# pujariaditya/WaveVerify

Hardware: AMD Instinct MI355X
Metric: clips/sec embed+detect, 1s@16kHz bs=256 (higher is better)
Workload: dtype f32; 1 GPU; embed_detect: 256 clips x 1 s @ 16 kHz per GPU (BASELINE.json configs[1]), seeded random weights; batch_per_gpu=256, global_batch=256, clip_samples=16000, parallelism=dp1 (independent clip shards, no data-path collective)

## Files before the change

include/waveverify_hip.h:

```cpp
#ifndef WAVEVERIFY_HIP_H
#define WAVEVERIFY_HIP_H

#include <stddef.h>
#include <stdint.h>

#ifdef __cplusplus
extern "C" {
#endif

#define WV_OK 0
#define WV_EINVAL (-1)
#define WV_ENOKEY (-2)
#define WV_EHIP (-3)
#define WV_ESTATE (-4)
#define WV_ENOMEM (-5)

#define WV_KIND_GENERATOR 0
#define WV_KIND_DETECTOR 1
#define WV_KIND_LOCATOR 2

#define WV_MAX_STRIDES 8

typedef struct wv_config {
    int32_t kind;
// ... 78 lines not shown
int wv_profile_collect(int index, char* name_out, int name_cap, int64_t* launches,
                       double* total_ms, double* flops, double* bytes);

int wv_window_gather(const float* src, int64_t n_src, const int64_t* offs, float* dst, int W, int L, void* stream);
int wv_window_scatter(const float* y, const int64_t* desc, float* out, int64_t n_out, int W, int C, int L, void* stream);
int wv_detector_forward_windowed(wv_model* m, const float* x, const int* keep_lo, const int* keep_hi, float* psum,
                                 int W, int L, void* workspace, size_t workspace_bytes, void* stream);
int wv_detector_forward_windowed_f16(wv_model* m, const float* x, const int* keep_lo, const int* keep_hi, float* psum,
                                     int W, int L, void* workspace, size_t workspace_bytes, void* stream);
int wv_window_reduce_mean(const float* psum, int n_rows, const int* ptr, const int* rows, const int64_t* lengths,
                          float* mean_prob, int B, int nb, void* stream);
int wv_frames_reduce(const float* fsum, int B, int nb, int Fr_stride, const int* seg, int n_seg, float eps, float* prob, double* count,
                     void* stream);
int wv_session_advance(const float* hist, int hcap, int hv, const float* x, int n, float* win, int wlen,
                       float* hist_out, int drop, int hv2, int S, void* stream);


int wv_op_pw_dw(const float* X, const float* w_pw, const float* w_dw, const float* dw_bias,
                const float* film, const float* resid, float* Y,
                int B, int K, int M, int Tin, int ks, int stride, int dilation,
                float pre_scale, int pre_elu, float out_scale, int bands,
                float* Yact, float act_scale, void* stream);

int wv_op_resblock(const float* X, float pre_scale, const float* w_pw1, const float* w_dw1, const float* b1,
                   const float* w_pw2, const float* w_dw2, const float* b2, float* Y, float* Yact,
                   int B, int C, int T, float out_scale, float act_scale, void* stream);

int wv_op_dw_pw(const float* X, const float* w_dw, const float* w_pw, const float* bias, float* Y,
                int B, int K, int M, int Tin, int mode, int ks_or_ratio,
                float pre_scale, int pre_elu, int l2norm, int accumulate, float out_scale,
                float* Yact, float act_scale, void* stream);

int wv_op_stft_logmag(const float* wav, const float* host_basis, float* P, int B, int T,
                      int n_fft, int hop, float mean, float std, void* stream);

int wv_op_spec_block(const float* wav, const float* basis_or_null, const float* w_pw, const float* x, float* Y, float* Yact, int B, int T,
                     int n_fft, int hop, int M, float mean, float std, float out_scale, float act_scale, void* stream);

int wv_op_conv_pre(const float* x, const float* w, const float* bias, float* Y, int B, int C,
                   int T, int ks, float in_scale, void* stream);

int wv_op_tail(const float* H, const float* w, const float* bias, const float* x_or_null,
               float* out, int B, int C, int Tin, int T, int ks, float pre_scale, float out_scale,
               void* stream);

int wv_op_head(const float* Z, const float* w_rev, const float* b_rev,
// ... 231 lines not shown
```

waveverify_amd/_lib.py:

```python
from __future__ import annotations

import ctypes as C
import os
from typing import Optional

HERE = os.path.dirname(os.path.abspath(__file__))
LIB_PATH = os.path.join(HERE, "lib", "libwaveverify_hip.so")
WV_MAX_STRIDES = 8

WV_KIND = {"generator": 0, "detector": 1, "locator": 2}


class WvConfig(C.Structure):
    _fields_ = [
        ("kind", C.c_int32), ("dimension", C.c_int32), ("msg_dimension", C.c_int32),
        ("channels_enc", C.c_int32), ("channels_dec", C.c_int32), ("n_fft_base", C.c_int32),
        ("n_residual_enc", C.c_int32), ("n_residual_dec", C.c_int32), ("n_strides", C.c_int32),
        ("strides", C.c_int32 * WV_MAX_STRIDES),
        ("kernel_size", C.c_int32), ("last_kernel_size", C.c_int32),
        ("residual_kernel_size", C.c_int32), ("dilation_base", C.c_int32),
        ("zero_init", C.c_int32), ("nbits", C.c_int32), ("output_dim", C.c_int32),
        ("embedding_dim", C.c_int32), ("embedding_layers", C.c_int32), ("freq_bands", C.c_int32),
        ("res_scale_enc", C.c_float), ("res_scale_dec", C.c_float), ("wav_std", C.c_float),
        ("spec_means", C.c_float * (WV_MAX_STRIDES + 1)),
# ... 10 lines not shown
    "wv_config_default": (C.c_int, [C.c_int, C.POINTER(WvConfig)]),
    "wv_model_create": (C.c_int, [C.POINTER(WvConfig), C.POINTER(_VP)]),
    "wv_model_destroy": (None, [_VP]),
    "wv_model_num_params": (C.c_int, [_VP]),
    "wv_model_param_info": (C.c_int, [_VP, C.c_int, C.c_char_p, C.c_int, C.POINTER(C.c_int64),
                                      C.POINTER(C.c_int), C.POINTER(C.c_int)]),
    "wv_model_set_param": (C.c_int, [_VP, C.c_char_p, _VP, C.c_int64]),
    "wv_model_set_param_wn": (C.c_int, [_VP, C.c_char_p, _VP, C.c_int64, _VP, C.c_int64]),
    "wv_model_set_stft_basis": (C.c_int, [_VP, C.c_char_p, _VP, C.c_int64]),
    "wv_model_finalize": (C.c_int, [_VP]),
    "wv_workspace_bytes": (C.c_size_t, [_VP, C.c_int, C.c_int]),
    "wv_generator_forward": (C.c_int, [_VP, _VP, _VP, C.c_int, _VP, C.c_int, C.c_int, C.c_int,
                                       _VP, C.c_size_t, _VP]),
    "wv_detector_forward": (C.c_int, [_VP, _VP, _VP, _VP, C.c_int, C.c_int, _VP, C.c_size_t, _VP]),
    "wv_locator_forward": (C.c_int, [_VP, _VP, _VP, C.c_int, C.c_int, _VP, C.c_size_t, _VP]),
    "wv_encoder_forward": (C.c_int, [_VP, _VP, _VP, C.c_int, _VP, C.c_int, C.c_int, _VP,
                                     C.c_size_t, _VP]),
    "wv_detector_forward_f16": (C.c_int, [_VP, _VP, _VP, _VP, C.c_int, C.c_int, _VP, C.c_size_t, _VP]),
    "wv_detector_forward_frames": (C.c_int, [_VP, _VP, _VP, C.c_float, _VP, C.c_int, C.c_int, _VP, C.c_size_t, _VP]),
    "wv_detector_forward_frames_f16": (C.c_int, [_VP, _VP, _VP, C.c_float, _VP, C.c_int, C.c_int, _VP, C.c_size_t, _VP]),
    "wv_locator_forward_f16": (C.c_int, [_VP, _VP, _VP, C.c_int, C.c_int, _VP, C.c_size_t, _VP]),
    "wv_generator_forward_f16": (C.c_int, [_VP, _VP, _VP, C.c_int, _VP, C.c_int, C.c_int, C.c_int, _VP, C.c_size_t, _VP]),
    "wv_model_film": (C.c_int, [_VP, _VP, C.c_int, _VP, C.c_int, _VP]),
    "wv_profile_enable": (C.c_int, [C.c_int]),
    "wv_profile_reset": (C.c_int, []),
    "wv_profile_collect": (C.c_int, [C.c_int, C.c_char_p, C.c_int, C.POINTER(C.c_int64),
                                     C.POINTER(C.c_double), C.POINTER(C.c_double),
                                     C.POINTER(C.c_double)]),
    "wv_window_gather": (C.c_int, [_VP, C.c_int64, _VP, _VP, C.c_int, C.c_int, _VP]),
    "wv_window_scatter": (C.c_int, [_VP, _VP, _VP, C.c_int64, C.c_int, C.c_int, C.c_int, _VP]),
    "wv_detector_forward_windowed": (C.c_int, [_VP, _VP, _VP, _VP, _VP, C.c_int, C.c_int, _VP, C.c_size_t, _VP]),
    "wv_detector_forward_windowed_f16": (C.c_int, [_VP, _VP, _VP, _VP, _VP, C.c_int, C.c_int, _VP, C.c_size_t, _VP]),
    "wv_window_reduce_mean": (C.c_int, [_VP, C.c_int, _VP, _VP, _VP, _VP, C.c_int, C.c_int, _VP]),
    "wv_frames_reduce": (C.c_int, [_VP, C.c_int, C.c_int, C.c_int, _VP, C.c_int, C.c_float, _VP, _VP, _VP]),
    "wv_session_advance": (C.c_int, [_VP, C.c_int, C.c_int, _VP, C.c_int, _VP, C.c_int, _VP, C.c_int, C.c_int, C.c_int, _VP]),
    "wv_op_pw_dw": (C.c_int, [_VP, _VP, _VP, _VP, _VP, _VP, _VP, C.c_int, C.c_int, C.c_int,
                              C.c_int, C.c_int, C.c_int, C.c_int, C.c_float, C.c_int, C.c_float,
                              C.c_int, _VP, C.c_float, _VP]),
    "wv_op_resblock": (C.c_int, [_VP, C.c_float] + [_VP] * 8 + [C.c_int, C.c_int, C.c_int, C.c_float, C.c_float, _VP]),
    "wv_op_dw_pw": (C.c_int, [_VP, _VP, _VP, _VP, _VP, C.c_int, C.c_int, C.c_int, C.c_int, C.c_int,
                              C.c_int, C.c_float, C.c_int, C.c_int, C.c_int, C.c_float, _VP, C.c_float, _VP]),
    "wv_op_stft_logmag": (C.c_int, [_VP, _VP, _VP, C.c_int, C.c_int, C.c_int, C.c_int, C.c_float,
                                    C.c_float, _VP]),
    "wv_op_spec_block": (C.c_int, [_VP] * 6 + [C.c_int] * 5 + [C.c_float] * 4 + [_VP]),
    "wv_op_conv_pre": (C.c_int, [_VP, _VP, _VP, _VP, C.c_int, C.c_int, C.c_int, C.c_int,
                                 C.c_float, _VP]),
# ... 174 lines not shown
```

waveverify_amd/csrc/wv_k1.hip:

```cpp
#include <algorithm>
#include <atomic>
#include <cstdlib>
#include <string>
#include <type_traits>

#include "wv_dev.h"

namespace wv {

typedef const __attribute__((address_space(1))) void* gptr_t;
typedef __attribute__((address_space(3))) void* lptr_t;

__device__ __attribute__((aligned(16))) float g_zero16[4] = {0.f, 0.f, 0.f, 0.f};

__device__ __forceinline__ float dpp_next(float v) {
    return __builtin_bit_cast(float, __builtin_amdgcn_update_dpp(0, __builtin_bit_cast(int, v), 0x130, 0xf, 0xf, true));
}

template <int NT_, int BKC_, int BM_ = 128>
struct K1 {
    static constexpr int NT = NT_, BN = 32 * NT_, BKC = BKC_, KQ = BKC_ / 4, BM = BM_, WM = BM_ / 32, NTHREADS = 64 * WM;
    static constexpr int A4 = KQ * BM;
    static constexpr int B4 = BKC * BN / 4;
    static constexpr int STAGE4 = A4 + B4;
    static constexpr int A_PIECES = A4 / 64, B_PIECES = B4 / 64;
    static constexpr int A_PER = (A_PIECES + WM - 1) / WM, B_PER_DMA = (B_PIECES + WM - 1) / WM;
    static constexpr int CG = BN / 4;
    static constexpr int HLD = BN + 4;
    static constexpr int NBT = (BKC / 2) * CG;
    static constexpr int B_PER = (NBT + NTHREADS - 1) / NTHREADS;
    static_assert(A4 % 64 == 0 && B4 % 64 == 0 && NTHREADS % CG == 0 && 64 % CG == 0, "staging maps");
};

template <int NT> struct NVec;
template <> struct NVec<4> { typedef f32x4 type; };
template <> struct NVec<2> { typedef f32x2 type; };

constexpr int OOB_VOFF = 0x40000000;

template <class C>
struct DmaRows {
    const float* src; size_t ld; int K; int rbase;
    __device__ __forceinline__ void init(const float* Xb, int K_, int Tin, int ti0, int wave, int lane) {
        const int col = ti0 + 4 * (lane % C::CG);
        rbase = lane / C::CG;
        const bool inr = col >= 0 && col + 3 < Tin;
        src = inr ? Xb + col : g_zero16;
        ld = inr ? (size_t)Tin : 0;
        K = K_;
        (void)wave;
    }
    __device__ __forceinline__ void init_flat(const float* X, int K_, int Tin, int B, int Tv, int pad, long long g0, int lane) {
        const long long g = g0 + 4 * (lane % C::CG);
        const int b = (int)(g / Tv), t = (int)(g - (long long)b * Tv) - pad;
        rbase = lane / C::CG;
        const bool inr = b < B && t >= 0;
        src = inr ? X + (size_t)b * K_ * Tin + t : g_zero16;
        ld = inr ? (size_t)Tin : 0;
        K = K_;
    }
    __device__ __forceinline__ void issue(int c, f32x4* Bst, int wave) const {
#pragma unroll
        for (int i = 0; i < C::B_PER_DMA; ++i) {
            const int pi = wave + i * C::WM;
            if (C::B_PIECES % C::WM == 0 || pi < C::B_PIECES) {
                const int k = min(c * C::BKC + pi * (64 / C::CG) + rbase, K - 1);
                __builtin_amdgcn_global_load_lds((gptr_t)(src + (size_t)k * ld), (lptr_t)(Bst + pi * 64), 16, 0, 0);
            }
        }
    }
};

template <class C>
struct DmaA {
    __amdgpu_buffer_rsrc_t rsrc;
    int voff[C::A_PER];
    int chunk_bytes;
    __device__ __forceinline__ void init(const f32x4* wq, int Mp, int m0, int nchunks, int wave, int lane) {
        rsrc = __builtin_amdgcn_make_buffer_rsrc(const_cast<f32x4*>(wq + m0), 0, (nchunks * C::KQ * Mp - m0) * 16, 0x00020000);
        chunk_bytes = C::KQ * Mp * 16;
#pragma unroll
        for (int i = 0; i < C::A_PER; ++i) {
            const int idx = (wave + i * C::WM) * 64 + lane;
            voff[i] = ((idx / C::BM) * Mp + idx % C::BM) * 16;
        }
    }
    __device__ __forceinline__ void issue(int c, f32x4* Ast, int wave) const {
        const int soff = c * chunk_bytes;
#pragma unroll
        for (int i = 0; i < C::A_PER; ++i) {
            const int pi = wave + i * C::WM;
// ... 82 lines not shown
        voff0 = act_lane ? ((m0 + 32 * wave + 4 * half) * p.Tout + to) * 4 : 0x7f000000;
        if (EPI == 0 && p.flat) {
            const long long gc = gflat + p.pad + o;
            const int bo2 = (int)(gc / p.Tv), t = (int)(gc - (long long)bo2 * p.Tv) - p.pad;
            const bool ok = o < p.tto && bo2 < p.B && t >= 0;
            Yb = p.Y; Ab = p.Yact; Rb = HASR ? p.resid : nullptr; Rb2 = RES == 2 ? p.resid2 : nullptr; Hb = RAWH ? p.Yraw : nullptr; Sb = RES == 5 ? p.Ysum : nullptr;
            nrec = (int)((long long)p.B * M * p.Tout * 4);
            voff0 = ok ? (int)((((long long)bo2 * M + m0 + 32 * wave + 4 * half) * p.Tout + t) * 4) : (int)0x80000000u;
        }
        if (EPI == 8 && p.flat) {
            const int TvO = p.Tv >> 3;
            const long long go = gflat / 8 + (q >> 1);
            const int bo2 = (int)(go / TvO), n = (int)(go - (long long)bo2 * TvO);
            const bool ok = (q & 1) == 0 && (q >> 1) < p.tto && bo2 < p.B && n < p.Tout;
            Yb = p.Y; Ab = p.Yact;
            nrec = (int)((long long)p.B * M * p.Tout * 4);
            voff0 = ok ? (int)((((long long)bo2 * M + m0 + 32 * wave + 4 * half) * p.Tout + n) * 4) : (int)0x80000000u;
            fgam = 1.f; fbet = 0.f;
            if (p.film) {
                const float* fl = p.film + (size_t)min(bo2, p.B - 1) * p.film_stride + 2 * (m0 / (M / p.bands));
                fgam = fl[0]; fbet = fl[1];
            }
        }
        const bool lane_film = EPI == 8 && p.flat;
        const int bw = p.film ? (M / p.bands) : 1;
        const float* filmb = (p.film && !lane_film) ? p.film + (size_t)b * p.film_stride : nullptr;
        for (int m = tid; m < C::BM; m += C::NTHREADS) {
            const int gm = m0 + m;
            float* row = Wl + m * WLD;
#pragma unroll
            for (int i = 0; i < NTAP; ++i) row[i] = (gm < M && i < p.ks) ? p.dw_w[(size_t)gm * p.ks + i] : 0.f;
            float gam = 1.f, bet = 0.f;
            if (filmb && gm < M) { const int band = gm / bw; gam = filmb[2 * band]; bet = filmb[2 * band + 1]; }
            row[NTAP] = (gm < M && p.dw_b) ? p.dw_b[gm] : 0.f;
            row[NTAP + 1] = gam; row[NTAP + 2] = bet;
            if (EPI != 0) row[WLD - 1] = 0.f;
        }
    }

    typedef unsigned uvec __attribute__((ext_vector_type(NT)));
    __device__ __forceinline__ ovec buf_load(__amdgpu_buffer_rsrc_t r, int off) const {
        if constexpr (NT == 4) return __builtin_bit_cast(ovec, __builtin_amdgcn_raw_buffer_load_b128(r, off, 0, 0));
        else return __builtin_bit_cast(ovec, __builtin_amdgcn_raw_buffer_load_b64(r, off, 0, 0));
    }
    __device__ __forceinline__ void buf_store(__amdgpu_buffer_rsrc_t r, int off, ovec v) const {
        if constexpr (NT == 4) __builtin_amdgcn_raw_buffer_store_b128(__builtin_bit_cast(uvec, v), r, off, 0, 0);
        else __builtin_amdgcn_raw_buffer_store_b64(__builtin_bit_cast(uvec, v), r, off, 0, 0);
    }

    __device__ __forceinline__ void finish(f32x16 (&acc)[NT], const PwDwArgs& p, float* strips) {
        if constexpr (EPI == 0) {
            constexpr int NSH = 4 / NT;
            const int clip_bytes = nrec;
            const __amdgpu_buffer_rsrc_t rY = uniform_rsrc(Yb ? Yb : p.Yact, Yb ? clip_bytes : 0);
            const __amdgpu_buffer_rsrc_t rA = uniform_rsrc(Ab ? Ab : p.Yact, Ab ? clip_bytes : 0);
            const __amdgpu_buffer_rsrc_t rR = uniform_rsrc(Rb ? Rb : p.X, Rb ? clip_bytes : 0);
            const int row_bytes = p.Tout * 4;
            const int voff = voff0;
            const float* Wrow = Wl + (32 * wave + 4 * half) * 8;
            ovec res4[HASR ? 4 : 1];
            ovec add4[RES == 2 ? 4 : 1];
            const __amdgpu_buffer_rsrc_t rR2 = uniform_rsrc(Rb2 ? Rb2 : p.X, Rb2 ? clip_bytes : 0);
            const __amdgpu_buffer_rsrc_t rH = uniform_rsrc(Hb ? Hb : p.Y, Hb ? clip_bytes : 0);
            const __amdgpu_buffer_rsrc_t rS = uniform_rsrc(Sb ? Sb : p.Y, Sb ? clip_bytes : 0);
            const float sres = (RES == 5 && p.scale_ptr) ? p.out_scale * p.scale_ptr[0] : p.out_scale;
            if constexpr (HASR) {
#pragma unroll
                for (int r = 0; r < 4; ++r) res4[r] = buf_load(rR, voff + ((r & 3) + 8 * (r >> 2)) * row_bytes);
            }
            if constexpr (RES == 2) {
#pragma unroll
                for (int r = 0; r < 4; ++r) add4[r] = buf_load(rR2, voff + ((r & 3) + 8 * (r >> 2)) * row_bytes);
            }
            f32x4 w0n = *reinterpret_cast<const f32x4*>(Wrow), w1n = *reinterpret_cast<const f32x4*>(Wrow + 4);
#pragma unroll
            for (int r = 0; r < 16; ++r) {
                const int cr = (r & 3) + 8 * (r >> 2);
                const f32x4 w0 = w0n, w1 = w1n;
                if (r + 1 < 16) {
                    const int cn = ((r + 1) & 3) + 8 * ((r + 1) >> 2);
                    w0n = *reinterpret_cast<const f32x4*>(Wrow + cn * 8);
                    w1n = *reinterpret_cast<const f32x4*>(Wrow + cn * 8 + 4);
                }
                float hh[NT + 4], cur[NT];
#pragma unroll
                for (int e = 0; e < NT; ++e) { cur[e] = acc[e][r]; hh[e] = cur[e]; }
#pragma unroll
                for (int s2 = 1; s2 <= NSH; ++s2) {
#pragma unroll
                    for (int e = 0; e < NT; ++e) { cur[e] = dpp_next(cur[e]); hh[s2 * NT + e] = cur[e]; }
                }
                const int off = voff + cr * row_bytes;
                ovec y;
#pragma unroll
                for (int e = 0; e < NT; ++e) {
                    float v = fmaf(w0.x, hh[e], w1.y);
// ... 157 lines not shown
template <> struct LdrSel<4> { typedef ConvTrPair<1> type; };
template <> struct LdrSel<5> { typedef ConvTrPair<0> type; };
template <> struct LdrSel<6> { typedef ConvTrLds<4> type; };
template <> struct LdrSel<7> { typedef ConvTrLds<2> type; };
template <class C> constexpr int k1_lwp(int ldr) { return ldr == 7 ? (C::BN / 2 + 6 + 3) / 4 * 4 : (C::BN / 4 + 6 + 3) / 4 * 4; }

template <class C, int EPI, int LDR, int RES, int NS>
__global__ __launch_bounds__(C::NTHREADS, LDR >= 2 ? (C::B_PER > 1 ? 2 : 3) : 4) void k1_kernel(PwDwArgs p) {
    extern __shared__ __attribute__((aligned(16))) float smem[];
    constexpr bool REG = LDR != 0;
    typedef K1Epi<C, EPI, RES> Epi;
    typedef typename LdrSel<LDR>::type LB;
    typedef typename NVec<C::NT>::type bvec;
    constexpr bool FLAT_OK = EPI == 0 || EPI == 8;
    TileId tile = decode_tile(p);
    if (FLAT_OK && p.flat) {
        const unsigned L = blockIdx.x, j = L >> 3;
        tile.m_tile = j % p.num_m; tile.t_tile = (j / p.num_m) * 8 + (L & 7); tile.b = 0;
        tile.valid = tile.t_tile < p.num_t;
    }
    if (!tile.valid) return;
    const long long gflat = (long long)tile.t_tile * p.tto * p.stride;
    f32x4* S4 = reinterpret_cast<f32x4*>(smem);
    float* table = smem + NS * C::STAGE4 * 4;
    static_assert(NS == 2 || (NS == 3 && LDR == 0), "three stages: DMA path only");
    const int tid = threadIdx.x, lane = tid & 63;
    const int wave = __builtin_amdgcn_readfirstlane(tid >> 6);
    const int h = lane >> 5, i31 = lane & 31;
    const int cg = tid % C::CG;
    const int K = p.pw.K, Mp = p.pw.Mp;
    const int nchunks = (K + C::BKC - 1) / C::BKC;
    const f32x4* wq = reinterpret_cast<const f32x4*>(p.pw.wq);
    const int m0 = tile.m_tile * C::BM, b = tile.b;
    const int to0 = tile.t_tile * p.tto;
    const int ti0 = to0 * p.stride - p.pad - p.off;
    const float* Xb = p.X + (size_t)b * K * p.Tin;

    constexpr int LWP = LDR >= 6 ? k1_lwp<C>(LDR) : 4;
    Epi epi;
    epi.begin(p, table, m0, b, to0, gflat);
    DmaRows<C> db{};
    DmaA<C> da;
    da.init(wq, Mp, m0, nchunks, wave, lane);
    LB lb{};
    float raw[REG ? C::B_PER : 1][REG ? LB::NRAW : 1];
    if constexpr (LDR == 0) {
        if (FLAT_OK && p.flat) db.init_flat(p.X, K, p.Tin, p.B, p.Tv, p.pad, gflat, lane);
        else db.init(Xb, K, p.Tin, ti0, wave, lane);
    }
    else {
        const float* Xt = Xb;
        int c0 = ti0, ncols = p.Tin, tout = p.Tout;
        if (EPI == 0 && p.flat) {
            const long long g = gflat + 4 * cg;
            const int bb = (int)(g / p.Tv), t = (int)(g - (long long)bb * p.Tv) - p.pad;
            const bool inb = bb < p.B;
            Xt = p.X + (size_t)(inb ? bb : 0) * K * p.Tin;
            c0 = t - 4 * cg; ncols = inb ? p.Tin : 0; tout = inb ? p.Tout : 0;
        }
        if constexpr (LDR == 1) lb = LB{Xt, K, p.Tin, ncols, c0, p.pre_scale, p.pre_elu, nullptr, 0, false, false};
        else if constexpr (LDR >= 6) {
            const int lfirst = max(c0, 0) / p.ratio;
            lb = LB{p.ct_w, K, p.ratio, c0, LWP, ((lfirst - 1) & ~3), C::BKC - 1, nullptr, 0, 0};
        }
        else lb = LB{Xt, p.ct_w, p.ct_wt, K, p.pw.Kp, p.Tin, tout, c0, p.ratio, p.pre_scale, p.pre_elu, 0, 0, {}, {}};
    }
    float* Rbuf = table + Epi::TABLE_FLOATS;
    auto issue_rows = [&](int c, int buf) {
        if constexpr (LDR >= 6) {
            constexpr int PPR = LWP / 4, NPIECE = C::BKC * PPR, NINST = (NPIECE + 63) / 64, PER = (NINST + C::WM - 1) / C::WM;
// ... 21 lines not shown
#pragma unroll
            for (int r = 0; r < C::B_PER; ++r) {
                const int idx = tid + r * C::NTHREADS;
                if (C::NBT % C::NTHREADS == 0 || idx < C::NBT) lb.fetch2(c * C::BKC + 2 * (idx / C::CG), raw[r]);
            }
        }
    };
    auto commit = [&](int c, int st) {
        if constexpr (LDR >= 6) lb.Rcur = Rbuf + (size_t)(c & 1) * C::BKC * LWP;
        if constexpr (REG) {
            f32x4* Bq = S4 + st * C::STAGE4 + C::A4;
#pragma unroll
            for (int r = 0; r < C::B_PER; ++r) {
                const int idx = tid + r * C::NTHREADS;
                if (!(C::NBT % C::NTHREADS == 0 || idx < C::NBT)) continue;
                const int kp = idx / C::CG;
                float o[8];
                lb.finish2(c * C::BKC + 2 * kp, raw[r], o);
                Bq[(2 * kp) * C::CG + cg] = f32x4{o[0], o[1], o[2], o[3]};
                Bq[(2 * kp + 1) * C::CG + cg] = f32x4{o[4], o[5], o[6], o[7]};
            }
        }
    };
    constexpr int PIECES_MIN = C::A_PIECES / C::WM + C::B_PIECES / C::WM;
    f32x16 acc[C::NT];
#pragma unroll
    for (int e = 0; e < C::NT; ++e)
#pragma unroll
        for (int r = 0; r < 16; ++r) acc[e][r] = 0.f;
    issue(0, 0);
    if constexpr (NS == 2) {
        if constexpr (LDR >= 6) {
            issue_rows(0, 0);
            __syncthreads();
        }
        if constexpr (REG) { lb.init(cg); fetch(0); commit(0, 0); }
        __syncthreads();
    } else {
        if (nchunks > 1) { issue(1, 1); asm volatile("s_waitcnt vmcnt(%0)" :: "n"(PIECES_MIN) : "memory"); }
        else asm volatile("s_waitcnt vmcnt(0)" ::: "memory");
        asm volatile("s_waitcnt lgkmcnt(0)" ::: "memory");
        __builtin_amdgcn_s_barrier();
    }
    int st = 0;
    for (int c = 0; c < nchunks; ++c) {
        const f32x4* S = S4 + st * C::STAGE4;
        const int stn = st + 1 == NS ? 0 : st + 1;
        if constexpr (NS == 2) {
            if (c + 1 < nchunks) { issue(c + 1, stn); fetch(c + 1); }
        } else {
            if (c + 2 < nchunks) issue(c + 2, stn + 1 == NS ? 0 : stn + 1);
        }
        const float* Bf = reinterpret_cast<const float*>(S + C::A4) + C::NT * i31;
#pragma unroll
        for (int g = 0; g < C::BKC / 16; ++g) {
            const f32x4 a0 = S[(4 * g + h) * C::BM + 32 * wave + i31];
            const f32x4 a1 = S[(4 * g + h + 2) * C::BM + 32 * wave + i31];
#define WV_K1_STEP(AV, ROW)                                                                        \
    { const bvec bv = *reinterpret_cast<const bvec*>(Bf + (ROW) * C::BN);                          \
      _Pragma("unroll") for (int e = 0; e < C::NT; ++e)                                            \
          acc[e] = __builtin_amdgcn_mfma_f32_32x32x2f32(AV, bv[e], acc[e], 0, 0, 0); }
            WV_K1_STEP(a0.x, 16 * g + 4 * h + 0) WV_K1_STEP(a0.y, 16 * g + 4 * h + 1)
            WV_K1_STEP(a0.z, 16 * g + 4 * h + 2) WV_K1_STEP(a0.w, 16 * g + 4 * h + 3)
            WV_K1_STEP(a1.x, 16 * g + 8 + 4 * h + 0) WV_K1_STEP(a1.y, 16 * g + 8 + 4 * h + 1)
            WV_K1_STEP(a1.z, 16 * g + 8 + 4 * h + 2) WV_K1_STEP(a1.w, 16 * g + 8 + 4 * h + 3)
#undef WV_K1_STEP
        }
        if constexpr (NS == 2) {
            if (c + 1 < nchunks) commit(c + 1, stn);
            __syncthreads();
        } else {
            if (c + 2 < nchunks) asm volatile("s_waitcnt vmcnt(%0)" :: "n"(PIECES_MIN) : "memory");
            else asm volatile("s_waitcnt vmcnt(0)" ::: "memory");
            __builtin_amdgcn_s_barrier();
        }
        st = stn;
    }
    epi.finish(acc, p, smem);
}

static bool aligned16(const void* p) { return (reinterpret_cast<uintptr_t>(p) & 15) == 0; }

bool k1_supported(const PwDwArgs& a) {
    if (!a.pw.wq || a.pw.Mp % 128) return false;
    if (a.pw.M < 33) return false;
    if (((a.ct_w ? a.Tout : a.Tin) & 3) || !aligned16(a.X) || a.pw.K < 1) return false;
    if ((long long)a.pw.K * a.Tin * 4 >= OOB_VOFF || (long long)a.pw.M * a.Tout * 4 >= OOB_VOFF) return false;
    if (a.Y && !aligned16(a.Y)) return false;
    if (a.Yact && !aligned16(a.Yact)) return false;
    if (a.resid && !aligned16(a.resid)) return false;
    if ((a.resid2 && !aligned16(a.resid2)) || (a.Yraw && !aligned16(a.Yraw)) || (a.Ysum && !aligned16(a.Ysum))) return false;
    if (a.ks < 1 || a.ks > 16 || (a.ks - 1) * a.dil + 1 + 3 > 64) return false;
    if (a.ct_w && a.ratio == 1) return false;
    return true;
}

template <class C, int EPI, int LDR, int RES, int NS = 2>
static hipError_t k1_run(PwDwArgs a, hipStream_t s, const char* base) {
    const size_t smem = NS * (size_t)C::STAGE4 * 16 + (size_t)K1Epi<C, EPI, RES>::TABLE_FLOATS * sizeof(float) +
                        (LDR >= 6 ? (size_t)2 * C::BKC * k1_lwp<C>(LDR) * sizeof(float) : 0);
    static_assert(C::WM * 4 * C::HLD <= 2 * C::STAGE4 * 4, "strips alias the stages");
    a.num_m = (a.pw.M + C::BM - 1) / C::BM;
    a.num_t = (a.Tout + a.tto - 1) / a.tto;
    a.stagger = 0; a.first_gen = 0;
    long long n_act = (long long)a.num_t * a.B;
    if (a.flat) {
        if (!(C::NT == 4 && (EPI == 0 || (EPI == 8 && LDR == 0)))) return hipErrorInvalidValue;
        n_act = EPI == 8 ? ((long long)a.B * (a.Tv / 8) + a.tto - 1) / a.tto : ((long long)a.B * a.Tv - a.pad + a.tto - 1) / a.tto;
        if (n_act > 0x7fffffffLL) return hipErrorInvalidValue;
        a.num_t = (int)n_act;
    }
    const long long nblk = ((n_act + 7) / 8) * 8 * a.num_m;
    if (nblk > 0x7fffffffLL) return hipErrorInvalidValue;
    std::string name;
    if (prof::enabled())
        name = std::string(base) + "<" + std::to_string(C::BM) + "," + std::to_string(C::BN) + (LDR == 0 ? (NS == 3 ? ",dma3" : ",dma") : (LDR >= 6 ? ",win" : ",reg")) + (a.flat ? ",flat>" : ">");
    const double M = a.pw.M, K = a.pw.K, Bd = a.B;
    const double outs = (a.Y ? 1.0 : 0.0) + (a.Yact ? 1.0 : 0.0) + (a.resid ? 1.0 : 0.0);
    const double flops = a.ct_w ? 2.0 * Bd * a.Tout * K * (M + 2.0) : 2.0 * Bd * M * (K * a.Tin + (double)a.ks * a.Tout);
    prof::Scope ps(s, name.c_str(), flops, 4.0 * Bd * (K * a.Tin + M * a.Tout * outs));
    hipLaunchKernelGGL((k1_kernel<C, EPI, LDR, RES, NS>), dim3((unsigned)nblk), dim3(C::NTHREADS), smem, s, a);
    return hipGetLastError();
}

bool pw_dw_geometry(PwDwArgs& a, int BN);

template <class C, int EPI, int RES>
static hipError_t k1_pick_ldr(const PwDwArgs& a, hipStream_t s) {
    if (a.ct_w) {
        if constexpr (EPI == 0 && RES == 0) {
#ifndef K1_NO_LDS_UPSAMPLE
            if (!a.flat && a.pre_scale == 1.f && !a.pre_elu && a.pw.K % C::BKC == 0 && a.Tin % 4 == 0 && a.Tout == a.Tin * a.ratio && C::BM <= 128) {
                if (a.ratio % 4 == 0) return k1_run<C, 0, 6, false>(a, s, "convtr_pw_lds");
                if (a.ratio == 2) return k1_run<C, 0, 7, false>(a, s, "convtr_pw_lds");
            }
#endif
            if (a.ratio % 4 == 0) return k1_run<C, 0, 2, false>(a, s, "convtr_pw");
            if (a.ratio == 2) return k1_run<C, 0, 3, false>(a, s, "convtr_pw");
            return k1_run<C, 0, 5, false>(a, s, "convtr_pw");
        }
        return hipErrorInvalidValue;
    }
    const char* base = a.spec_add ? "spec_add" : (EPI == 0 ? (RES == 2 ? "pw_dw_k5_dact" : RES == 4 ? "pw_dw_k5_h" : RES == 5 ? "pw_dw_k5_hres" : RES ? "pw_dw_k5" : "pw_dw_k5_nr") : (EPI == 1 ? "pw_dw" : "pw_dw_s"));
    if (a.pre_elu || a.pre_scale != 1.f) return k1_run<C, EPI, 1, RES>(a, s, base);
    if constexpr (C::NT == 4 && C::BM == 128) {
        if (EPI == 0 && a.pw.K >= 256) return k1_run<C, EPI, 0, RES, 3>(a, s, base);
    }
    return k1_run<C, EPI, 0, RES>(a, s, base);
}

template <class C>
static hipError_t k1_pick_epi(const PwDwArgs& a, hipStream_t s, bool k5) {
    const bool res = a.resid != nullptr;
    if (a.res_mode == 2) {
        if (!k5 || !res) return hipErrorNotSupported;
        return k1_pick_ldr<C, 0, 2>(a, s);
    }
    if (a.Yraw) {
        if (!k5 || a.ct_w || (res != (a.Ysum != nullptr))) return hipErrorNotSupported;
        return res ? k1_pick_ldr<C, 0, 5>(a, s) : k1_pick_ldr<C, 0, 4>(a, s);
    }
    if (k5) return res ? k1_pick_ldr<C, 0, true>(a, s) : k1_pick_ldr<C, 0, false>(a, s);
    if constexpr (C::NT == 4) {
        if (!res && !a.ct_w && a.dil == 1 && a.ks == 2 * a.stride && a.pad == a.stride &&
            a.off == (a.stride == 2 ? 2 : 0)) {
            if (a.stride == 2) return k1_pick_ldr<C, 2, false>(a, s);
            if (a.stride == 4) return k1_pick_ldr<C, 4, false>(a, s);
            if (a.stride == 8) return k1_pick_ldr<C, 8, false>(a, s);
        }
// ... 369 lines not shown
```

waveverify_amd/csrc/wv_kernels.h:

```cpp
#pragma once
#include <hip/hip_runtime.h>
#include <stdint.h>

#include <cstring>
#include <vector>

namespace wv {

constexpr int BK = 16;
constexpr int M_ALIGN = 128;

inline int round_up(int x, int a) { return (x + a - 1) / a * a; }

struct PwWeight {
    const float* wt = nullptr;
    int K = 0, M = 0, Kp = 0, Mp = 0;
    const float* wq = nullptr;
};
struct PwDwArgs {
    const float* X;
    PwWeight pw;
    const float* dw_w;
    const float* dw_b;
    const float* film;
// ... 3 lines not shown
    float* Ysum;
    const float* scale_ptr;
    int res_mode;
    float* Y;
    int B, Tin, Tout, ks, stride, dil, pad;
    float pre_scale;
    int pre_elu;
    float out_scale;
    int bands, film_stride;
    float* Yact;
    float act_scale;
    int num_m, num_t;
    int stagger, first_gen;
    int tto, off;
    int spec_add;
    int flat, Tv;
    const float* ct_w;
    int ratio;
    const float* ct_wt;
};
hipError_t launch_pw_dw(const PwDwArgs& a, hipStream_t s);
bool k1_supported(const PwDwArgs& a);
hipError_t launch_k1(const PwDwArgs& a, hipStream_t s);
bool pw_dw_geometry(PwDwArgs& a, int BN);
struct RbArgs {
    const float* X;
    float pre_scale;
    PwWeight pw1, pw2;
    const float* tab1;
    const float* tab2;
    float* Y;
    float* Yact;
    float out_scale, act_scale;
    int B, C, T;
    int num_t, ntiles;
    const float* out_scale_ptr = nullptr;
    float *sv_h0 = nullptr, *sv_u = nullptr, *sv_h1 = nullptr, *sv_v = nullptr;
};
bool rb_supported(const RbArgs& a);
hipError_t launch_resblock(const RbArgs& a, hipStream_t s);
inline std::vector<float> pack_rb_table(const float* dw_w, const float* dw_b, int C) {
    std::vector<float> t((size_t)C * 8, 0.f);
    for (int m = 0; m < C; ++m) {
        for (int i = 0; i < 5; ++i) t[(size_t)m * 8 + i] = dw_w[(size_t)m * 5 + i];
        t[(size_t)m * 8 + 5] = dw_b ? dw_b[m] : 0.f;
        t[(size_t)m * 8 + 6] = 1.f;
// ... 282 lines not shown
```

waveverify_amd/csrc/wv_ops.hip:

```cpp
#include <hip/hip_runtime.h>

#include <cmath>
#include <cstring>
#include <string>
#include <vector>

#include "wv_host.h"
#include "wv_kernels.h"

namespace {

using wv::al256;
using wv::fail;

struct Tmp {
    std::vector<void*> d;
    bool ok = true;
    const float* up(const float* h, size_t n) {
        if (!h || !ok) return nullptr;
        void* p = nullptr;
        if (hipMalloc(&p, std::max<size_t>(n, 1) * sizeof(float)) != hipSuccess) { ok = false; return nullptr; }
        d.push_back(p);
        if (n && hipMemcpy(p, h, n * sizeof(float), hipMemcpyHostToDevice) != hipSuccess) { ok = false; return nullptr; }
        return (const float*)p;
// ... 60 lines not shown
        bc[n] = (float)acc;
    }
}

}

extern "C" {

int wv_op_pw_dw(const float* X, const float* w_pw, const float* w_dw, const float* dw_bias,
                const float* film, const float* resid, float* Y, int B, int K, int M, int Tin,
                int ks, int stride, int dilation, float pre_scale, int pre_elu, float out_scale,
                int bands, float* Yact, float act_scale, void* stream) {
    if (!X || !w_pw || !w_dw || (!Y && !Yact) || B < 1 || K < 1 || M < 1 || Tin < 1) return fail(WV_EINVAL, "null pointer (X, w_pw, w_dw, or both Y and Yact) or B, K, M, Tin < 1");
    Tmp t;
    wv::PwDwArgs a{};
    a.X = X; a.pw = t.pw(w_pw, M, K); a.dw_w = t.up(w_dw, (size_t)M * ks);
    a.dw_b = t.up(dw_bias, M); a.film = film; a.resid = resid; a.Y = Y; a.Yact = Yact; a.act_scale = act_scale;
    a.B = B; a.Tin = Tin; a.Tout = (Tin + stride - 1) / stride; a.ks = ks; a.stride = stride;
    a.dil = dilation; a.pad = (ks - 1) * dilation - (stride - 1);
    a.pre_scale = pre_scale; a.pre_elu = pre_elu; a.out_scale = out_scale;
    a.bands = bands > 0 ? bands : 1; a.film_stride = 2 * a.bands;
    if (a.pad < 0) return fail(WV_EINVAL, "negative left pad: (ks - 1) * dilation < stride - 1");
    return done(t, wv::launch_pw_dw(a, (hipStream_t)stream), (hipStream_t)stream);
}

int wv_op_resblock(const float* X, float pre_scale, const float* w_pw1, const float* w_dw1, const float* b1,
                   const float* w_pw2, const float* w_dw2, const float* b2, float* Y, float* Yact,
                   int B, int C, int T, float out_scale, float act_scale, void* stream) {
    if (!X || !w_pw1 || !w_dw1 || !w_pw2 || !w_dw2 || (!Y && !Yact) || B < 1 || C < 1 || T < 1) return fail(WV_EINVAL, "null pointer (X, a weight, or both Y and Yact) or B, C, T < 1");
    Tmp t;
    wv::RbArgs a{};
    a.X = X; a.pre_scale = pre_scale; a.pw1 = t.pw(w_pw1, C, C); a.pw2 = t.pw(w_pw2, C, C);
    a.tab1 = t.upv(wv::pack_rb_table(w_dw1, b1, C)); a.tab2 = t.upv(wv::pack_rb_table(w_dw2, b2, C));
    a.Y = Y; a.Yact = Yact; a.out_scale = out_scale; a.act_scale = act_scale; a.B = B; a.C = C; a.T = T;
    const hipError_t e = wv::launch_resblock(a, (hipStream_t)stream);
    if (e == hipErrorNotSupported) return unsupported(std::string("C in {64, 96, 128, 192}, T % 4 == 0") + FUSED_GATES);
    return done(t, e, (hipStream_t)stream);
}

int wv_h16_round_host(const float* in, uint16_t* out, int64_t n) {
    if (!in || !out || n < 0) return fail(WV_EINVAL, "null pointer or n < 0");
    for (int64_t i = 0; i < n; ++i) out[i] = wv::f32_to_f16_bits(in[i]);
    return WV_OK;
}
int wv_h16_from_f32(const float* X, void* Y16, int B, int C, int T, float scale, int elu, void* stream) {
    Tmp t;
// ... 423 lines not shown
```

Baseline: 3470 clips/s.

## Replace three-stage k1 pipeline with A2/B3 split staging and late table fill

Replaces the three-full-stage DMA pipeline in the pointwise/depthwise GEMM kernel with a plan that double-buffers the weight tile (A) and triple-buffers the activation tile (B). The epilogue row table and strips now alias the dead stages and are filled late, which shrinks LDS to fit four workgroups per CU. The plan is also extended to the EPI==8 (film) variant. B row pointers are now precomputed and advanced by a fixed step instead of recomputing addresses with a clamp each chunk. It adds an occupancy query entry point, and the late table fill adds a barrier in the epilogue.

```diff
diff --git a/include/waveverify_hip.h b/include/waveverify_hip.h
--- a/include/waveverify_hip.h
+++ b/include/waveverify_hip.h
@@ -124,6 +124,8 @@
                 float pre_scale, int pre_elu, float out_scale, int bands,
                 float* Yact, float act_scale, void* stream);
 
+int wv_k1_plan_occupancy(int* blocks_per_cu, int* lds_bytes);
+
 int wv_op_resblock(const float* X, float pre_scale, const float* w_pw1, const float* w_dw1, const float* b1,
                    const float* w_pw2, const float* w_dw2, const float* b2, float* Y, float* Yact,
                    int B, int C, int T, float out_scale, float act_scale, void* stream);
diff --git a/waveverify_amd/_lib.py b/waveverify_amd/_lib.py
--- a/waveverify_amd/_lib.py
+++ b/waveverify_amd/_lib.py
@@ -56,6 +56,7 @@
     "wv_locator_forward_f16": (C.c_int, [_VP, _VP, _VP, C.c_int, C.c_int, _VP, C.c_size_t, _VP]),
     "wv_generator_forward_f16": (C.c_int, [_VP, _VP, _VP, C.c_int, _VP, C.c_int, C.c_int, C.c_int, _VP, C.c_size_t, _VP]),
     "wv_model_film": (C.c_int, [_VP, _VP, C.c_int, _VP, C.c_int, _VP]),
+    "wv_k1_plan_occupancy": (C.c_int, [C.POINTER(C.c_int), C.POINTER(C.c_int)]),
     "wv_profile_enable": (C.c_int, [C.c_int]),
     "wv_profile_reset": (C.c_int, []),
     "wv_profile_collect": (C.c_int, [C.c_int, C.c_char_p, C.c_int, C.POINTER(C.c_int64),
diff --git a/waveverify_amd/csrc/wv_k1.hip b/waveverify_amd/csrc/wv_k1.hip
--- a/waveverify_amd/csrc/wv_k1.hip
+++ b/waveverify_amd/csrc/wv_k1.hip
@@ -32,6 +32,9 @@
     static_assert(A4 % 64 == 0 && B4 % 64 == 0 && NTHREADS % CG == 0 && 64 % CG == 0, "staging maps");
 };
 
+constexpr int NS_A2B3 = 5;
+template <class C> constexpr int k1_plan_bytes() { return (2 * C::A4 + 3 * C::B4) * 16; }
+
 template <int NT> struct NVec;
 template <> struct NVec<4> { typedef f32x4 type; };
 template <> struct NVec<2> { typedef f32x2 type; };
@@ -40,33 +43,51 @@
 
 template <class C>
 struct DmaRows {
-    const float* src; size_t ld; int K; int rbase;
+    const float* src; unsigned ld; int K; int rbase;
+    const float* row[C::B_PER_DMA];
+    unsigned step;
+    __device__ __forceinline__ void start(int wave) {
+#pragma unroll
+        for (int i = 0; i < C::B_PER_DMA; ++i) row[i] = src + (size_t)((wave + i * C::WM) * (64 / C::CG) + rbase) * ld;
+        step = (unsigned)C::BKC * ld * 4u;
+    }
     __device__ __forceinline__ void init(const float* Xb, int K_, int Tin, int ti0, int wave, int lane) {
         const int col = ti0 + 4 * (lane % C::CG);
         rbase = lane / C::CG;
         const bool inr = col >= 0 && col + 3 < Tin;
         src = inr ? Xb + col : g_zero16;
-        ld = inr ? (size_t)Tin : 0;
+        ld = inr ? (unsigned)Tin : 0u;
         K = K_;
-        (void)wave;
-    }
-    __device__ __forceinline__ void init_flat(const float* X, int K_, int Tin, int B, int Tv, int pad, long long g0, int lane) {
+        start(wave);
+    }
+    __device__ __forceinline__ void init_flat(const float* X, int K_, int Tin, int B, int Tv, int pad, long long g0, int wave, int lane) {
         const long long g = g0 + 4 * (lane % C::CG);
         const int b = (int)(g / Tv), t = (int)(g - (long long)b * Tv) - pad;
         rbase = lane / C::CG;
         const bool inr = b < B && t >= 0;
         src = inr ? X + (size_t)b * K_ * Tin + t : g_zero16;
-        ld = inr ? (size_t)Tin : 0;
+        ld = inr ? (unsigned)Tin : 0u;
         K = K_;
-    }
-    __device__ __forceinline__ void issue(int c, f32x4* Bst, int wave) const {
+        start(wave);
+    }
+    __device__ __forceinline__ void issue(int c, f32x4* Bst, int wave) {
+        if ((c + 1) * C::BKC > K) {
+#pragma unroll
+            for (int i = 0; i < C::B_PER_DMA; ++i) {
+                const int pi = wave + i * C::WM;
+                if (C::B_PIECES % C::WM == 0 || pi < C::B_PIECES) {
+                    const int k = min(c * C::BKC + pi * (64 / C::CG) + rbase, K - 1);
+                    __builtin_amdgcn_global_load_lds((gptr_t)(src + (size_t)k * ld), (lptr_t)(Bst + pi * 64), 16, 0, 0);
+                }
+            }
+            return;
+        }
 #pragma unroll
         for (int i = 0; i < C::B_PER_DMA; ++i) {
             const int pi = wave + i * C::WM;
-            if (C::B_PIECES % C::WM == 0 || pi < C::B_PIECES) {
-                const int k = min(c * C::BKC + pi * (64 / C::CG) + rbase, K - 1);
-                __builtin_amdgcn_global_load_lds((gptr_t)(src + (size_t)k * ld), (lptr_t)(Bst + pi * 64), 16, 0, 0);
-            }
+            if (C::B_PIECES % C::WM == 0 || pi < C::B_PIECES)
+                __builtin_amdgcn_global_load_lds((gptr_t)row[i], (lptr_t)(Bst + pi * 64), 16, 0, 0);
+            row[i] = reinterpret_cast<const float*>(reinterpret_cast<const char*>(row[i]) + step);
         }
     }
 };
@@ -195,20 +216,34 @@
                 fgam = fl[0]; fbet = fl[1];
             }
         }
+    }
+    __device__ __forceinline__ void fill_table(const PwDwArgs& p) {
+        const int tid = threadIdx.x;
         const bool lane_film = EPI == 8 && p.flat;
         const int bw = p.film ? (M / p.bands) : 1;
         const float* filmb = (p.film && !lane_film) ? p.film + (size_t)b * p.film_stride : nullptr;
         for (int m = tid; m < C::BM; m += C::NTHREADS) {
-            const int gm = m0 + m;
+            const int gm = m0 + m, gc = min(gm, M - 1);
+            const bool in = gm < M;
             float* row = Wl + m * WLD;
-#pragma unroll
-            for (int i = 0; i < NTAP; ++i) row[i] = (gm < M && i < p.ks) ? p.dw_w[(size_t)gm * p.ks + i] : 0.f;
-            float gam = 1.f, bet = 0.f;
-            if (filmb && gm < M) { const int band = gm / bw; gam = filmb[2 * band]; bet = filmb[2 * band + 1]; }
-            row[NTAP] = (gm < M && p.dw_b) ? p.dw_b[gm] : 0.f;
-            row[NTAP + 1] = gam; row[NTAP + 2] = bet;
+            const float* wrow = p.dw_w + (size_t)gc * p.ks;
+            float tap[NTAP];
+#pragma unroll
+            for (int i = 0; i < NTAP; ++i) tap[i] = wrow[min(i, p.ks - 1)];
+            float bias = 0.f, gam = 1.f, bet = 0.f;
+            if (p.dw_b) bias = p.dw_b[gc];
+            if (filmb) { const int band = gc / bw; gam = filmb[2 * band]; bet = filmb[2 * band + 1]; }
+#pragma unroll
+            for (int i = 0; i < NTAP; ++i) row[i] = (in && i < p.ks) ? tap[i] : 0.f;
+            row[NTAP] = in ? bias : 0.f;
+            row[NTAP + 1] = in ? gam : 1.f; row[NTAP + 2] = in ? bet : 0.f;
             if (EPI != 0) row[WLD - 1] = 0.f;
         }
+    }
+    __device__ __forceinline__ void late_table(const PwDwArgs& p) {
+        fill_table(p);
+        asm volatile("s_waitcnt lgkmcnt(0)" ::: "memory");
+        __builtin_amdgcn_s_barrier();
     }
 
     typedef unsigned uvec __attribute__((ext_vector_type(NT)));
@@ -221,7 +256,9 @@
         else __builtin_amdgcn_raw_buffer_store_b64(__builtin_bit_cast(uvec, v), r, off, 0, 0);
     }
 
+    template <bool LATE>
     __device__ __forceinline__ void finish(f32x16 (&acc)[NT], const PwDwArgs& p, float* strips) {
+        if constexpr (LATE && EPI != 0) late_table(p);
         if constexpr (EPI == 0) {
             constexpr int NSH = 4 / NT;
             const int clip_bytes = nrec;
@@ -237,6 +274,7 @@
             const __amdgpu_buffer_rsrc_t rH = uniform_rsrc(Hb ? Hb : p.Y, Hb ? clip_bytes : 0);
             const __amdgpu_buffer_rsrc_t rS = uniform_rsrc(Sb ? Sb : p.Y, Sb ? clip_bytes : 0);
             const float sres = (RES == 5 && p.scale_ptr) ? p.out_scale * p.scale_ptr[0] : p.out_scale;
+            if constexpr (LATE && RES == 2) late_table(p);
             if constexpr (HASR) {
 #pragma unroll
                 for (int r = 0; r < 4; ++r) res4[r] = buf_load(rR, voff + ((r & 3) + 8 * (r >> 2)) * row_bytes);
@@ -245,6 +283,7 @@
 #pragma unroll
                 for (int r = 0; r < 4; ++r) add4[r] = buf_load(rR2, voff + ((r & 3) + 8 * (r >> 2)) * row_bytes);
             }
+            if constexpr (LATE && RES != 2) late_table(p);
             f32x4 w0n = *reinterpret_cast<const f32x4*>(Wrow), w1n = *reinterpret_cast<const f32x4*>(Wrow + 4);
 #pragma unroll
             for (int r = 0; r < 16; ++r) {
@@ -448,8 +487,12 @@
     if (!tile.valid) return;
     const long long gflat = (long long)tile.t_tile * p.tto * p.stride;
     f32x4* S4 = reinterpret_cast<f32x4*>(smem);
-    float* table = smem + NS * C::STAGE4 * 4;
-    static_assert(NS == 2 || (NS == 3 && LDR == 0), "three stages: DMA path only");
+    constexpr bool PLAN = NS == NS_A2B3;
+    static_assert(NS == 2 || (PLAN && LDR == 0), "A2/B3 plan: DMA path only");
+    static_assert(!PLAN || (C::A_PIECES % C::WM == 0 && C::B_PIECES % C::WM == 0), "A2/B3 plan: the counted wait needs the same piece count in every wave");
+    static_assert(!PLAN || k1_plan_bytes<C>() <= 40960, "A2/B3 plan: four workgroups per CU (4 x 40 KiB = 160 KiB)");
+    static_assert(!PLAN || ((EPI == 1 || EPI == 5 ? C::WM * 4 * C::HLD : 0) + Epi::TABLE_FLOATS) * 4 <= k1_plan_bytes<C>(), "A2/B3 plan: strips and row table share the dead stages");
+    float* table = PLAN ? smem + k1_plan_bytes<C>() / 4 - Epi::TABLE_FLOATS : smem + NS * C::STAGE4 * 4;
     const int tid = threadIdx.x, lane = tid & 63;
     const int wave = __builtin_amdgcn_readfirstlane(tid >> 6);
     const int h = lane >> 5, i31 = lane & 31;
@@ -465,13 +508,14 @@
     constexpr int LWP = LDR >= 6 ? k1_lwp<C>(LDR) : 4;
     Epi epi;
     epi.begin(p, table, m0, b, to0, gflat);
+    if constexpr (!PLAN) epi.fill_table(p);
     DmaRows<C> db{};
     DmaA<C> da;
     da.init(wq, Mp, m0, nchunks, wave, lane);
     LB lb{};
     float raw[REG ? C::B_PER : 1][REG ? LB::NRAW : 1];
     if constexpr (LDR == 0) {
-        if (FLAT_OK && p.flat) db.init_flat(p.X, K, p.Tin, p.B, p.Tv, p.pad, gflat, lane);
+        if (FLAT_OK && p.flat) db.init_flat(p.X, K, p.Tin, p.B, p.Tv, p.pad, gflat, wave, lane);
         else db.init(Xb, K, p.Tin, ti0, wave, lane);
     }
     else {
@@ -539,36 +583,41 @@
             }
         }
     };
-    constexpr int PIECES_MIN = C::A_PIECES / C::WM + C::B_PIECES / C::WM;
     f32x16 acc[C::NT];
 #pragma unroll
     for (int e = 0; e < C::NT; ++e)
 #pragma unroll
         for (int r = 0; r < 16; ++r) acc[e][r] = 0.f;
-    issue(0, 0);
-    if constexpr (NS == 2) {
+    constexpr int B_MINE = C::B_PIECES / C::WM;
+    auto issue_a = [&](int c) { da.issue(c, S4 + (c & 1) * C::A4, wave); };
+    auto issue_b = [&](int c, int sb) { db.issue(c, S4 + 2 * C::A4 + sb * C::B4, wave); };
+    if constexpr (PLAN) {
+        issue_a(0); issue_b(0, 0);
+        if (nchunks > 1) { issue_b(1, 1); asm volatile("s_waitcnt vmcnt(%0)" :: "n"(B_MINE) : "memory"); }
+        else asm volatile("s_waitcnt vmcnt(0)" ::: "memory");
+        __builtin_amdgcn_s_barrier();
+    } else {
+        issue(0, 0);
         if constexpr (LDR >= 6) {
             issue_rows(0, 0);
             __syncthreads();
         }
         if constexpr (REG) { lb.init(cg); fetch(0); commit(0, 0); }
         __syncthreads();
-    } else {
-        if (nchunks > 1) { issue(1, 1); asm volatile("s_waitcnt vmcnt(%0)" :: "n"(PIECES_MIN) : "memory"); }
-        else asm volatile("s_waitcnt vmcnt(0)" ::: "memory");
-        asm volatile("s_waitcnt lgkmcnt(0)" ::: "memory");
-        __builtin_amdgcn_s_barrier();
-    }
+    }
+    constexpr int NSB = PLAN ? 3 : 2;
     int st = 0;
     for (int c = 0; c < nchunks; ++c) {
-        const f32x4* S = S4 + st * C::STAGE4;
-        const int stn = st + 1 == NS ? 0 : st + 1;
-        if constexpr (NS == 2) {
+        const f32x4* S = PLAN ? S4 + (c & 1) * C::A4 : S4 + st * C::STAGE4;
+        const f32x4* SB = PLAN ? S4 + 2 * C::A4 + st * C::B4 : S4 + st * C::STAGE4 + C::A4;
+        const int stn = st + 1 == NSB ? 0 : st + 1;
+        if constexpr (PLAN) {
+            if (c + 1 < nchunks) issue_a(c + 1);
+            if (c + 2 < nchunks) issue_b(c + 2, stn + 1 == NSB ? 0 : stn + 1);
+        } else {
             if (c + 1 < nchunks) { issue(c + 1, stn); fetch(c + 1); }
-        } else {
-            if (c + 2 < nchunks) issue(c + 2, stn + 1 == NS ? 0 : stn + 1);
-        }
-        const float* Bf = reinterpret_cast<const float*>(S + C::A4) + C::NT * i31;
+        }
+        const float* Bf = reinterpret_cast<const float*>(SB) + C::NT * i31;
 #pragma unroll
         for (int g = 0; g < C::BKC / 16; ++g) {
             const f32x4 a0 = S[(4 * g + h) * C::BM + 32 * wave + i31];
@@ -583,17 +632,17 @@
             WV_K1_STEP(a1.z, 16 * g + 8 + 4 * h + 2) WV_K1_STEP(a1.w, 16 * g + 8 + 4 * h + 3)
 #undef WV_K1_STEP
         }
-        if constexpr (NS == 2) {
+        if constexpr (PLAN) {
+            if (c + 2 < nchunks) asm volatile("s_waitcnt vmcnt(%0)" :: "n"(B_MINE) : "memory");
+            else asm volatile("s_waitcnt vmcnt(0)" ::: "memory");
+            __builtin_amdgcn_s_barrier();
+        } else {
             if (c + 1 < nchunks) commit(c + 1, stn);
             __syncthreads();
-        } else {
-            if (c + 2 < nchunks) asm volatile("s_waitcnt vmcnt(%0)" :: "n"(PIECES_MIN) : "memory");
-            else asm volatile("s_waitcnt vmcnt(0)" ::: "memory");
-            __builtin_amdgcn_s_barrier();
         }
         st = stn;
     }
-    epi.finish(acc, p, smem);
+    epi.template finish<PLAN>(acc, p, smem);
 }
 
 static bool aligned16(const void* p) { return (reinterpret_cast<uintptr_t>(p) & 15) == 0; }
@@ -614,8 +663,9 @@
 
 template <class C, int EPI, int LDR, int RES, int NS = 2>
 static hipError_t k1_run(PwDwArgs a, hipStream_t s, const char* base) {
-    const size_t smem = NS * (size_t)C::STAGE4 * 16 + (size_t)K1Epi<C, EPI, RES>::TABLE_FLOATS * sizeof(float) +
-                        (LDR >= 6 ? (size_t)2 * C::BKC * k1_lwp<C>(LDR) * sizeof(float) : 0);
+    const size_t smem = NS == NS_A2B3 ? (size_t)k1_plan_bytes<C>()
+                                      : NS * (size_t)C::STAGE4 * 16 + (size_t)K1Epi<C, EPI, RES>::TABLE_FLOATS * sizeof(float) +
+                                            (LDR >= 6 ? (size_t)2 * C::BKC * k1_lwp<C>(LDR) * sizeof(float) : 0);
     static_assert(C::WM * 4 * C::HLD <= 2 * C::STAGE4 * 4, "strips alias the stages");
     a.num_m = (a.pw.M + C::BM - 1) / C::BM;
     a.num_t = (a.Tout + a.tto - 1) / a.tto;
@@ -631,13 +681,19 @@
     if (nblk > 0x7fffffffLL) return hipErrorInvalidValue;
     std::string name;
     if (prof::enabled())
-        name = std::string(base) + "<" + std::to_string(C::BM) + "," + std::to_string(C::BN) + (LDR == 0 ? (NS == 3 ? ",dma3" : ",dma") : (LDR >= 6 ? ",win" : ",reg")) + (a.flat ? ",flat>" : ">");
+        name = std::string(base) + "<" + std::to_string(C::BM) + "," + std::to_string(C::BN) + (LDR == 0 ? (EPI == 0 && NS == NS_A2B3 ? ",dma3" : ",dma") : (LDR >= 6 ? ",win" : ",reg")) + (a.flat ? ",flat>" : ">");
     const double M = a.pw.M, K = a.pw.K, Bd = a.B;
     const double outs = (a.Y ? 1.0 : 0.0) + (a.Yact ? 1.0 : 0.0) + (a.resid ? 1.0 : 0.0);
     const double flops = a.ct_w ? 2.0 * Bd * a.Tout * K * (M + 2.0) : 2.0 * Bd * M * (K * a.Tin + (double)a.ks * a.Tout);
     prof::Scope ps(s, name.c_str(), flops, 4.0 * Bd * (K * a.Tin + M * a.Tout * outs));
     hipLaunchKernelGGL((k1_kernel<C, EPI, LDR, RES, NS>), dim3((unsigned)nblk), dim3(C::NTHREADS), smem, s, a);
     return hipGetLastError();
+}
+
+hipError_t k1_plan_occupancy(int* blocks_per_cu, int* lds_bytes) {
+    typedef K1<4, 16, 128> C;
+    *lds_bytes = k1_plan_bytes<C>();
+    return hipOccupancyMaxActiveBlocksPerMultiprocessor(blocks_per_cu, k1_kernel<C, 0, 0, 1, NS_A2B3>, C::NTHREADS, (size_t)*lds_bytes);
 }
 
 bool pw_dw_geometry(PwDwArgs& a, int BN);
@@ -660,8 +716,8 @@
     }
     const char* base = a.spec_add ? "spec_add" : (EPI == 0 ? (RES == 2 ? "pw_dw_k5_dact" : RES == 4 ? "pw_dw_k5_h" : RES == 5 ? "pw_dw_k5_hres" : RES ? "pw_dw_k5" : "pw_dw_k5_nr") : (EPI == 1 ? "pw_dw" : "pw_dw_s"));
     if (a.pre_elu || a.pre_scale != 1.f) return k1_run<C, EPI, 1, RES>(a, s, base);
-    if constexpr (C::NT == 4 && C::BM == 128) {
-        if (EPI == 0 && a.pw.K >= 256) return k1_run<C, EPI, 0, RES, 3>(a, s, base);
+    if constexpr (C::NT == 4 && C::BM == 128 && (EPI == 0 || EPI == 8)) {
+        if (EPI == 8 || a.pw.K >= 256) return k1_run<C, EPI, 0, RES, NS_A2B3>(a, s, base);
     }
     return k1_run<C, EPI, 0, RES>(a, s, base);
 }
diff --git a/waveverify_amd/csrc/wv_kernels.h b/waveverify_amd/csrc/wv_kernels.h
--- a/waveverify_amd/csrc/wv_kernels.h
+++ b/waveverify_amd/csrc/wv_kernels.h
@@ -49,6 +49,7 @@
 hipError_t launch_pw_dw(const PwDwArgs& a, hipStream_t s);
 bool k1_supported(const PwDwArgs& a);
 hipError_t launch_k1(const PwDwArgs& a, hipStream_t s);
+hipError_t k1_plan_occupancy(int* blocks_per_cu, int* lds_bytes);
 bool pw_dw_geometry(PwDwArgs& a, int BN);
 struct RbArgs {
     const float* X;
diff --git a/waveverify_amd/csrc/wv_ops.hip b/waveverify_amd/csrc/wv_ops.hip
--- a/waveverify_amd/csrc/wv_ops.hip
+++ b/waveverify_amd/csrc/wv_ops.hip
@@ -106,6 +106,12 @@
     a.bands = bands > 0 ? bands : 1; a.film_stride = 2 * a.bands;
     if (a.pad < 0) return fail(WV_EINVAL, "negative left pad: (ks - 1) * dilation < stride - 1");
     return done(t, wv::launch_pw_dw(a, (hipStream_t)stream), (hipStream_t)stream);
+}
+
+int wv_k1_plan_occupancy(int* blocks_per_cu, int* lds_bytes) {
+    if (!blocks_per_cu || !lds_bytes) return fail(WV_EINVAL, "wv_k1_plan_occupancy: null pointer");
+    WV_HIP_TRY(wv::k1_plan_occupancy(blocks_per_cu, lds_bytes));
+    return WV_OK;
 }
 
 int wv_op_resblock(const float* X, float pre_scale, const float* w_pw1, const float* w_dw1, const float* b1,
```

After: 3469 clips/s. No clear change (-0.0%).
